# jank324/lynx

Hardware: AMD Instinct MI355X
Metric: particle-element-steps/sec (whole node) + achieved HBM GB/s, Segment.track ParticleBeam (higher is better)
Workload: dtype f32

## Files before the change

### lynx_amd/csrc/lynx_hip.hip

```cpp
#include <hip/hip_runtime.h>
#include <hip/hip_ext.h>
#include <rccl/rccl.h>

#include <algorithm>
#include <cstdio>
#include <cstdlib>
#include <cstring>
#include <map>
#include <mutex>
#include <string>
#include <type_traits>
#include <unordered_map>
#include <vector>

#include "lynx_device.hpp"
#include "lynx_grad.hpp"
#include "lynx_units.hpp"
#include "lynx_grad_units.hpp"
#include "lynx_trace.hpp"
#include "lynx_trace_grad.hpp"

using namespace lynx;

struct Knobs {
  int xpose = -1;
  int unroll = -1;
  int mom = -1;
  int min_tiles_per_wg = -1;
  int async_build = -1;
  int side_reduce = -1;
  int build_host_wait = -1;
  int gather_overlap = -1;
  int lanes_build_min_batch = 256;
  int piece = 8;
  int pair_levels_fused = 1;
  int merge_steps = 1;
  int reduce_ticket = 1;
  int one_round = -1;
  int track_units = 1;
  int unit_pairs = 1;
  int bwd_units = 1;
  int bwd_merge = 1;
  int bwd_pairs = 1;
  int build_in_tail = 1;
  int small_inline = -1;
  int bwd_reuse_table = 1;
  int host_visible_records = 1;
  int alternate_order = 1;
  int inline_pool = 1;
};

static void load_knobs(Knobs* k) {
  *k = Knobs();
  const struct { const char* name; int* value; } table[] = {
      {"LYNX_XPOSE", &k->xpose}, {"LYNX_UNROLL", &k->unroll}, {"LYNX_MOM", &k->mom},
      {"LYNX_MIN_TILES_PER_WG", &k->min_tiles_per_wg}, {"LYNX_ASYNC_BUILD", &k->async_build},
      {"LYNX_SIDE_REDUCE", &k->side_reduce}, {"LYNX_BUILD_HOST_WAIT", &k->build_host_wait},
      {"LYNX_GATHER_OVERLAP", &k->gather_overlap}, {"LYNX_LANES_BUILD_MIN_BATCH", &k->lanes_build_min_batch},
      {"LYNX_PIECE", &k->piece}, {"LYNX_PAIR_LEVELS_FUSED", &k->pair_levels_fused},
      {"LYNX_MERGE_STEPS", &k->merge_steps},
      {"LYNX_REDUCE_TICKET", &k->reduce_ticket}, {"LYNX_TRACK_UNITS", &k->track_units}, {"LYNX_ONE_ROUND", &k->one_round}, {"LYNX_UNIT_PAIRS", &k->unit_pairs}, {"LYNX_BWD_UNITS", &k->bwd_units},
      {"LYNX_BWD_MERGE", &k->bwd_merge}, {"LYNX_BWD_PAIRS", &k->bwd_pairs}, {"LYNX_BUILD_IN_TAIL", &k->build_in_tail},
      {"LYNX_SMALL_INLINE", &k->small_inline}, {"LYNX_INLINE_POOL", &k->inline_pool}, {"LYNX_ALTERNATE_ORDER", &k->alternate_order}, {"LYNX_HOST_VISIBLE_RECORDS", &k->host_visible_records}, {"LYNX_BWD_REUSE_TABLE", &k->bwd_reuse_table}};
  for (const auto& t : table) {
    const char* v = getenv(t.name);
    if (v && *v) *t.value = atoi(v);
  }
}
static inline int knob(int value, int dflt) { return value >= 0 ? value : dflt; }

struct lynx_ctx {
  Knobs knobs;
  int device = 0;
  hipStream_t stream = nullptr;
  hipStream_t s_build = nullptr;
  static constexpr int kTableSlots = 3;
  hipEvent_t ev_built[kTableSlots] = {}, ev_streamed_own[kTableSlots] = {}, ev_mark = nullptr;
  hipEvent_t ev_streamed[kTableSlots] = {};
  bool streamed_valid[kTableSlots] = {};
  unsigned seq = 0;
  bool main_dirty = false;
  bool main_idle = true;
  bool plain_events = false;
  unsigned long_calls = 0;
  struct FwdTable {
    const lynx_lattice* lat = nullptr;
    uint64_t version = 0;
    const void* energy = nullptr;
    int slot = -1;
    int merged = 0;
    bool units = false;
    size_t energy_bytes = 0;
    unsigned seq = 0;
    bool valid = false;
    void written(const void* dst, size_t bytes) {
      const char *a = (const char*)dst, *e = (const char*)energy;
      if (valid && a < e + energy_bytes && a + bytes > e) valid = false;
    }
  } fwd_table;
  const void* main_wrote = nullptr;
  std::mutex mu;
  void wrote(const void* dst, size_t bytes) {
    if (!dst || bytes == 0) return;
    std::lock_guard<std::mutex> lock(mu);
    fwd_table.written(dst, bytes);
  }
  hipEvent_t ev_start = nullptr, ev_stop = nullptr;
  int32_t* h_status = nullptr;
  int32_t* d_status = nullptr;
  unsigned int* d_tail_flag = nullptr;
  uint32_t tail_seq = 0;
  int can_wait_value = 0;
  std::string err;
  hipDeviceProp_t prop;
  std::multimap<size_t, void*> free_blocks;
  std::unordered_map<void*, size_t> live;
  std::vector<std::pair<const char*, size_t>> host_ranges;
  void* scratch_level = nullptr;
  size_t scratch_level_bytes = 0;
  unsigned int* scratch_tickets = nullptr;
  size_t scratch_tickets_count = 0;
  void* scratch_obs = nullptr;
  size_t scratch_obs_bytes = 0;
  void* scratch_erun = nullptr;
  size_t scratch_erun_bytes = 0;
  void* scratch_esteps = nullptr;
  size_t scratch_esteps_bytes = 0;
  int32_t* d_spec_valid = nullptr;
  void* scratch_products = nullptr;
  size_t scratch_products_bytes = 0;
  void* scratch_coefs = nullptr;
  size_t scratch_coefs_bytes = 0;
  static constexpr int kTableBwd = kTableSlots, kTablePb = kTableSlots + 1, kTableTrace = kTableSlots + 2;
  void* scratch_steps[kTableSlots + 3] = {};
  size_t scratch_steps_bytes[kTableSlots + 3] = {};
  void* scratch_trace[2] = {nullptr, nullptr};
  size_t scratch_trace_bytes[2] = {0, 0};
  void* scratch_trace_plan = nullptr;
  size_t scratch_trace_plan_bytes = 0;
  std::vector<int64_t> trace_plan;
  void* scratch_units_bwd[2] = {nullptr, nullptr};
  size_t scratch_units_bwd_bytes[2] = {0, 0};
  void* scratch_units[2 * kTableSlots] = {};
  size_t scratch_units_bytes[2 * kTableSlots] = {};
// ... 1014 lines not shown
      hipLaunchKernelGGL(k_pair_products, dim3((unsigned)groups, (unsigned)level.second), dim3(64), 0, stream,
                         lat->d_tasks + level.first, lat->batch, Bp, (double*)ctx->scratch_products);
      HIP_TRY(ctx, hipGetLastError());
    }
  }
  hipLaunchKernelGGL(k_emit_steps<T>, dim3((unsigned)groups, (unsigned)lat->n_steps), dim3(64), emit_steps_lds<T>(), stream, lv,
                     lat->d_step_slot, (const T*)d_energy_in, Bp, (const double*)ctx->scratch_products,
                     (const T*)ctx->scratch_coefs, merge_pairs, (T*)d_steps_out, (T*)d_energy_out,
                     d_units ? lat->d_step_unit[merge_pairs ? 1 : 0] : (const int32_t*)nullptr,
                     lat->units[merge_pairs ? 1 : 0].n_units, d_units, d_extras, se);
  HIP_TRY(ctx, hipGetLastError());
  return LYNX_OK;
}

template <typename T>
static int launch_build(lynx_ctx* ctx, lynx_lattice* lat, hipStream_t stream, const void* d_energy_in,
                        void* d_steps_out, void* d_energy_out, int merge_pairs = 0, bool underneath = false,
                        float* d_units = nullptr, float* d_extras = nullptr, bool force_lanes = false) {
  const bool lanes = lat->n_steps > 0 && (force_lanes || lat->batch >= ctx->knobs.lanes_build_min_batch);
  {
    const int rc = launch_cavity_flags<T>(ctx, lat, stream, d_energy_in, lanes);
    if (rc) return rc;
  }
  if (lanes) {
    const int rc = sync_pool(ctx, lat);
    return rc ? rc : launch_build_lanes<T>(ctx, lat, stream, d_energy_in, d_steps_out, d_energy_out, merge_pairs, d_units, d_extras);
  }
  int threads, chunk;
  build_shape<T>(ctx, lat, underneath, &threads, &chunk);
  const size_t lds = build_scratch_bytes(chunk, sizeof(T)) +
                     ((size_t)lat->n_steps * LYNX_STEP_STRIDE + lat->n_steps + 1) * sizeof(T);
  int rc;
  if (lat->prog_pool && ctx->knobs.inline_pool) {
    if ((size_t)lat->pool_count * sizeof(T) <= (size_t)kInlinePoolSmall) {
      if ((rc = allow_lds(ctx, k_build_inline<T, kInlinePoolSmall>, lds))) return rc;
      hipLaunchKernelGGL((k_build_inline<T, kInlinePoolSmall>), dim3((unsigned)lat->batch), dim3((unsigned)threads), lds, stream,
                         *reinterpret_cast<const InlinePool<kInlinePoolSmall>*>(&lat->h_pool), dev_view(lat),
                         (const T*)d_energy_in, (T*)d_steps_out, (T*)d_energy_out, chunk, merge_pairs);
    } else {
      if ((rc = allow_lds(ctx, k_build_inline<T, kInlinePoolLarge>, lds))) return rc;
      hipLaunchKernelGGL((k_build_inline<T, kInlinePoolLarge>), dim3((unsigned)lat->batch), dim3((unsigned)threads), lds, stream,
                         lat->h_pool, dev_view(lat), (const T*)d_energy_in, (T*)d_steps_out, (T*)d_energy_out, chunk, merge_pairs);
    }
  } else {
    if ((rc = sync_pool(ctx, lat)) || (rc = allow_lds(ctx, k_build<T>, lds))) return rc;
    hipLaunchKernelGGL(k_build<T>, dim3((unsigned)lat->batch), dim3((unsigned)threads), lds, stream, dev_view(lat),
                       (const T*)d_energy_in, (T*)d_steps_out, (T*)d_energy_out, chunk, merge_pairs);
  }
  HIP_TRY(ctx, hipGetLastError());
  if constexpr (sizeof(T) == 4) {
    if (d_units) {
      const UnitPlan& up = lat->units[merge_pairs ? 1 : 0];
      const int64_t n = lat->batch * up.n_units;
      hipLaunchKernelGGL(k_pack_units, dim3((unsigned)((n + 255) / 256)), dim3(256), 0, stream, up, lat->batch,
                         lat->n_steps, (const float*)d_steps_out, d_units, d_extras);
      HIP_TRY(ctx, hipGetLastError());
    }
  }
  return LYNX_OK;
}

int lynx_build_compose(lynx_ctx* ctx, lynx_lattice* lat, const void* d_energy_in, void* d_steps_out,
                       void* d_energy_out) {
  LYNX_NEED(ctx);
  ctx->main_idle = false;
  if (!ctx || !lat || !d_energy_in || !d_steps_out) return fail(ctx, LYNX_ERR_INVALID, "null argument");
  if (lat->batch > 0x7fffffffLL) return fail(ctx, LYNX_ERR_INVALID, "batch too large");
  HIP_TRY(ctx, use_device(ctx));
  ctx->main_dirty = true;
  const size_t es = dtype_size(lat->dtype);
  ctx->wrote(d_steps_out, (size_t)lat->batch * lat->n_steps * LYNX_STEP_STRIDE * es);
  ctx->wrote(d_energy_out, (size_t)lat->batch * es);
  return lat->dtype == LYNX_F64 ? launch_build<double>(ctx, lat, ctx->stream, d_energy_in, d_steps_out, d_energy_out)
                                : launch_build<float>(ctx, lat, ctx->stream, d_energy_in, d_steps_out, d_energy_out);
}


struct TrackPlan {
  hipEvent_t done = nullptr;
  bool full_cov;
  int unroll;
  int mom_mode;
  bool xpose;
  TrackArgs a;
  size_t lds;
  unsigned grid;
};

template <typename T>
static TrackPlan plan_track(lynx_ctx* ctx, const lynx_lattice* lat, int64_t B, int64_t N, int32_t S, bool moments,
                            bool full_cov) {
  TrackPlan p;
  p.full_cov = full_cov;
  constexpr int P = 16 / (int)sizeof(T);
  const int64_t cus = ctx->prop.multiProcessorCount > 0 ? ctx->prop.multiProcessorCount : 256;
  const Knobs& kn = ctx->knobs;
  const int64_t target = 512 * cus;
  p.mom_mode = knob(kn.mom, sizeof(T) == 4 ? 2 : 1);
  if (sizeof(T) == 8 || p.mom_mode < 2 || p.mom_mode > 3) p.mom_mode = sizeof(T) == 4 ? 2 : 1;
  p.a.n_particles = N;
  p.a.store = 0;
  p.a.tail_flag = nullptr;
  p.a.tail_seq = 0;
  p.a.tail_wg = 0;
  p.a.stash_offset = 0;
  p.a.reversed = 0;
  const bool single_map = S == 1 && lat && lat->h_steps[0].kind == LYNX_STEP_RUN &&
                          !(lat->h_steps[0].flags & LYNX_STEP_FLAG_OBSERVE);
  p.xpose = knob(kn.xpose, ((sizeof(T) == 8 || (single_map && !full_cov)) && N >= 8 * 64 * P) ? 1 : 0) != 0;
  int u = knob(kn.unroll, p.xpose ? P : (sizeof(T) == 4 ? (S > 1 ? 2 : 4) : 1));
  if (u != 1 && u != 2 && u != 4) u = 2;
  if (sizeof(T) == 8 && u > 2) u = 2;
  while (u > 1 && B * ((N + 256 * u - 1) / (256 * u)) < 4 * cus) u >>= 1;
  if (u != P) p.xpose = false;
  p.unroll = u;
  const int64_t tile = 256 * (int64_t)u;
  const int64_t ntiles = (N + tile - 1) / tile;
  int64_t min_tpw = std::max(1, knob(kn.min_tiles_per_wg, S > 1 ? 16 : 2));
  while (min_tpw > 1 && B * ((ntiles + min_tpw - 1) / min_tpw) < 4 * cus) --min_tpw;
  int64_t chunks = std::max<int64_t>(1, std::min<int64_t>((ntiles + min_tpw - 1) / min_tpw, (target + B - 1) / B));
  {
    const int64_t one_round = 3 * cus;
    const int cap = knob(kn.one_round, (S <= 1 && B * chunks > one_round && B * chunks <= 4 * one_round) ? 3 : 0);
    if (cap > 0) chunks = std::max<int64_t>(1, std::min<int64_t>(chunks, cap * cus / B));
  }
  int64_t tpw = (ntiles + chunks - 1) / chunks;
  chunks = (ntiles + tpw - 1) / tpw;
  p.a.chunks = (int32_t)chunks;
  p.a.tiles_per_wg = (int32_t)tpw;
  if (p.mom_mode == 2 && kn.mom < 0 && tpw * u <= 32) p.mom_mode = 3;
  if (p.mom_mode == 3 && tpw * u > 64) p.mom_mode = 2;
  size_t scratch = 4 * kPartialStride * sizeof(double);
  if (moments)
    scratch = std::max<size_t>(scratch, (size_t)(full_cov ? kMomSlabScalars : kMomSlabScalarsCompact) * (p.mom_mode >= 2 ? 4 : 8));
  if (p.xpose) scratch = std::max<size_t>(scratch, (size_t)(kTrackThreads / 64) * kWaveTileBytes);
  scratch = (scratch + 15) / 16 * 16;
  p.a.lds_scratch_bytes = (int32_t)scratch;
  p.a.n_observers = lat ? lat->n_observers : 0;
  p.lds = (scratch + ((size_t)S * LYNX_STEP_STRIDE + S + 1) * sizeof(T) + 7) / 8 * 8 + (size_t)2 * p.a.n_observers * 256 * sizeof(double);
  p.grid = (unsigned)(B * chunks);
  return p;
}

template <typename K, typename... Args>
static int launch_streaming(lynx_ctx* ctx, const TrackPlan& p, K kernel, size_t lds, const Args&... args) {
  int rc = allow_lds(ctx, kernel, lds);
  if (rc) return rc;
  hipEvent_t e0 = nullptr, e1 = p.done;
  if (ctx->profiling) {
    HIP_TRY(ctx, hipEventCreateWithFlags(&e0, timing_event_flags(ctx)));
    HIP_TRY(ctx, hipEventCreateWithFlags(&e1, timing_event_flags(ctx)));
  }
  hipExtLaunchKernelGGL(kernel, dim3(p.grid), dim3(kTrackThreads), (std::uint32_t)lds, ctx->stream, e0, e1, 0u, args...);
  HIP_TRY(ctx, hipGetLastError());
  if (ctx->profiling) ctx->prof_events.emplace_back(e0, e1);
  ctx->last_stream_stop = e1;
  return LYNX_OK;
}

template <typename T, int MOM, bool FULL, int UNROLL, bool XPOSE>
static int launch_direct_inst(lynx_ctx* ctx, const TrackPlan& p, const LatticeDev& lv, const void* d_energy_in,
                              const void* d_p_in, void* d_p_out, void* d_energy_out, const void* d_steps,
                              double* d_partials, double* d_obs) {
  return launch_streaming(ctx, p, k_track_direct<T, MOM, FULL, UNROLL, XPOSE>, p.lds, lv, p.a, (const T*)d_energy_in,
                          (const T*)d_p_in, (T*)d_p_out, (T*)d_energy_out, (const T*)d_steps, d_partials, d_obs);
}

#define LYNX_LAUNCH_ARGS ctx, p, lv, d_energy_in, d_p_in, d_p_out, d_energy_out, d_steps, d_partials, d_obs
#define LYNX_LAUNCH_PARAMS                                                                                     \
  lynx_ctx *ctx, const TrackPlan &p, const LatticeDev &lv, const void *d_energy_in, const void *d_p_in,        \
      void *d_p_out, void *d_energy_out, const void *d_steps, double *d_partials, double *d_obs

template <typename T, int MOM, bool FULL, int U>
static int launch_direct_mu(LYNX_LAUNCH_PARAMS) {
  if constexpr (U * 7 * sizeof(T) == 112) {
    if (p.xpose) return launch_direct_inst<T, MOM, FULL, U, true>(LYNX_LAUNCH_ARGS);
  }
  return launch_direct_inst<T, MOM, FULL, U, false>(LYNX_LAUNCH_ARGS);
}

template <typename T, int MOM, bool FULL>
static int launch_direct_m(LYNX_LAUNCH_PARAMS) {
  switch (p.unroll) {
    case 1: return launch_direct_mu<T, MOM, FULL, 1>(LYNX_LAUNCH_ARGS);
    case 2: return launch_direct_mu<T, MOM, FULL, 2>(LYNX_LAUNCH_ARGS);
    default:
      if constexpr (sizeof(T) == 4) return launch_direct_mu<T, MOM, FULL, 4>(LYNX_LAUNCH_ARGS);
      else return fail(ctx, LYNX_ERR_INVALID, "float64: at most 2 particles per lane");
  }
}

template <typename T>
static int launch_direct(LYNX_LAUNCH_PARAMS, bool moments) {
  const int mom = moments ? p.mom_mode : 0;
  if (mom == 0) return launch_direct_m<T, 0, false>(LYNX_LAUNCH_ARGS);
  if constexpr (sizeof(T) == 4) {
    if (mom == 3) return p.full_cov ? launch_direct_m<T, 3, true>(LYNX_LAUNCH_ARGS) : launch_direct_m<T, 3, false>(LYNX_LAUNCH_ARGS);
    return p.full_cov ? launch_direct_m<T, 2, true>(LYNX_LAUNCH_ARGS) : launch_direct_m<T, 2, false>(LYNX_LAUNCH_ARGS);
  } else {
    return p.full_cov ? launch_direct_m<T, 1, true>(LYNX_LAUNCH_ARGS) : launch_direct_m<T, 1, false>(LYNX_LAUNCH_ARGS);
  }
}
#undef LYNX_LAUNCH_ARGS
#undef LYNX_LAUNCH_PARAMS


static int proposed_class(const lynx_lattice* lat, int32_t first, int32_t last) {
  int rank = 1;
  for (int32_t e = first; e < last; ++e) {
    const lynx_elem& el = lat->h_elems[e];
    switch (el.kind) {
      case LYNX_KIND_IDENTITY:
      case LYNX_KIND_DRIFT:
      case LYNX_KIND_HCOR:
      case LYNX_KIND_VCOR:
      case LYNX_KIND_CAVITY:
      case LYNX_KIND_UNDULATOR: break;
      case LYNX_KIND_QUADRUPOLE: rank = std::max(rank, (el.flags & LYNX_FLAG_TILT) ? 3 : 1); break;
      case LYNX_KIND_DIPOLE: rank = std::max(rank, 2); break;
      default: rank = 3; break;
    }
  }
  return rank == 1 ? kClassU : rank == 2 ? kClassD : kClassDense;
}

static bool plan_units(const lynx_lattice* lat, bool merged, UnitPlan* plan) {
  const int32_t S = lat->n_steps;
  plan->n_units = 0;
  for (int32_t s = 0; s < S; ++s) {
    const lynx_step& st = lat->h_steps[s];
    if (st.flags & LYNX_STEP_FLAG_OBSERVE) return false;
    const bool pair = merged && s + 1 < S && st.kind == LYNX_STEP_RUN && lat->h_steps[s + 1].kind == LYNX_STEP_CAVITY;
    const int32_t last = pair ? lat->h_steps[s + 1].last : st.last;
    if (pair) ++s;
    if (plan->n_units >= kMaxUnits || s > 255) return false;
    const int u = plan->n_units++;
    plan->slot[u] = (unsigned char)s;
    plan->pair[u] = pair ? 1 : 0;
    plan->cls[u] = (unsigned char)proposed_class(lat, st.first, last);
  }
  for (int u = plan->n_units; u < kMaxUnits; ++u) plan->slot[u] = plan->cls[u] = plan->pair[u] = 0;
  return plan->n_units > 0;
}

static int ensure_units_plan(lynx_ctx* ctx, lynx_lattice* lat, bool merged) {
  const int m = merged ? 1 : 0;
  if (lat->units_made[m]) return LYNX_OK;
  UnitPlan& up = lat->units[m];
  lat->units_ok[m] = plan_units(lat, merged, &up) && lat->batch * up.n_units * kUnitStride < 0x7fffffffLL;
  lat->units_made[m] = true;
  if (!lat->units_ok[m]) return LYNX_OK;
  std::vector<int32_t> code((size_t)lat->n_steps, -1);
  for (int u = 0; u < up.n_units; ++u) code[up.slot[u]] = step_unit_code(u, up.cls[u], up.pair[u]);
  int rc;
  if (!lat->d_step_unit[m] && (rc = ctx_alloc(ctx, code.size() * sizeof(int32_t), (void**)&lat->d_step_unit[m]))) return rc;
  HIP_TRY(ctx, hipStreamSynchronize(ctx->s_build));
  HIP_TRY(ctx, sync_main(ctx));
  HIP_TRY(ctx, hipMemcpy(lat->d_step_unit[m], code.data(), code.size() * sizeof(int32_t), hipMemcpyHostToDevice));
  return LYNX_OK;
}

template <int MOM, bool FULL, int PAIRS, bool PAIR_FORM = false>
static int launch_units_inst(lynx_ctx* ctx, const TrackPlan& p, int32_t U, int32_t S, const void* d_p_in, void* d_p_out,
                             void* d_energy_out, const void* d_steps, const void* d_units, const void* d_extras,
                             double* d_partials) {
  const size_t lds = units_lds_bytes((size_t)p.a.lds_scratch_bytes, U);
  auto kernel = k_track_units<MOM, FULL, PAIRS>;
  if constexpr (PAIR_FORM) kernel = k_track_unit_pairs<MOM, FULL>;
  return launch_streaming(ctx, p, kernel, lds, p.a, U, S, (const float*)d_p_in, (float*)d_p_out, (float*)d_energy_out,
                          (const float*)d_steps, (const float*)d_units, (const float*)d_extras, d_partials);
}

static int launch_units(lynx_ctx* ctx, const TrackPlan& p, int32_t U, int32_t S, const void* d_p_in, void* d_p_out,
                        void* d_energy_out, const void* d_steps, const void* d_units, const void* d_extras,
                        double* d_partials, bool moments, bool pair_form) {
#define LYNX_UNITS_ARGS ctx, p, U, S, d_p_in, d_p_out, d_energy_out, d_steps, d_units, d_extras, d_partials
  if (pair_form)
    return moments ? launch_units_inst<3, false, 1, true>(LYNX_UNITS_ARGS) : launch_units_inst<0, false, 1, true>(LYNX_UNITS_ARGS);
  if (p.unroll == 4) {
    if (!moments) return launch_units_inst<0, false, 2>(LYNX_UNITS_ARGS);
    if (p.mom_mode == 3) return p.full_cov ? launch_units_inst<3, true, 2>(LYNX_UNITS_ARGS) : launch_units_inst<3, false, 2>(LYNX_UNITS_ARGS);
    return p.full_cov ? launch_units_inst<2, true, 2>(LYNX_UNITS_ARGS) : launch_units_inst<2, false, 2>(LYNX_UNITS_ARGS);
  }
  if (!moments) return launch_units_inst<0, false, 1>(LYNX_UNITS_ARGS);
  if (p.mom_mode == 3) return p.full_cov ? launch_units_inst<3, true, 1>(LYNX_UNITS_ARGS) : launch_units_inst<3, false, 1>(LYNX_UNITS_ARGS);
  return p.full_cov ? launch_units_inst<2, true, 1>(LYNX_UNITS_ARGS) : launch_units_inst<2, false, 1>(LYNX_UNITS_ARGS);
#undef LYNX_UNITS_ARGS
}

struct TrackTable {
  int slot = -1;
  bool async = false;
  bool tail = false;
  bool short_call = false;
  const void* d_steps = nullptr;
  const void* d_units = nullptr;
  const void* d_extras = nullptr;
  int n_units = 0;
  bool use_units = false;
};

template <typename T>
static int track_table(lynx_ctx* ctx, lynx_lattice* lat, int64_t B, int64_t N, int32_t S, const void* d_energy_in,
                       const void* d_energy_out, int flags, TrackPlan& p, TrackTable* t) {
  int rc;
  const int slot = t->slot = (int)(ctx->seq++ % (unsigned)lynx_ctx::kTableSlots);
  const size_t need = (size_t)B * S * LYNX_STEP_STRIDE * sizeof(T);
  if ((rc = ensure_scratch(ctx, &ctx->scratch_steps[slot], &ctx->scratch_steps_bytes[slot], need))) return rc;
  bool has_pair = false;
  for (int32_t s = 1; s < S; ++s)
    has_pair |= lat->h_steps[s].kind == LYNX_STEP_CAVITY && lat->h_steps[s - 1].kind == LYNX_STEP_RUN &&
                !(lat->h_steps[s - 1].flags & LYNX_STEP_FLAG_OBSERVE);
  p.a.merged_pairs = has_pair && sizeof(T) == 4 && p.unroll == 2 &&
                     !(flags & LYNX_TRACK_SEQUENTIAL_STEPS) && ctx->knobs.merge_steps;
  if (p.a.merged_pairs) {
    p.lds = (p.lds + 15) / 16 * 16;
    p.a.stash_offset = (int32_t)p.lds;
    p.lds += (size_t)kTrackThreads * 4 * sizeof(float);
  }
  const bool half_million = B * N >= (int64_t)512 << 10;
  t->short_call = half_million && (size_t)B * N * 7 * sizeof(T) < ((size_t)128 << 20) && !lat->has_cavity;
  bool inline_all = false;
  if (t->short_call && ctx->knobs.async_build < 0)
    inline_all = knob(ctx->knobs.small_inline, ctx->main_idle ? 1 : 0) != 0;
  const bool async = t->async = knob(ctx->knobs.async_build, half_million && !inline_all ? 1 : 0) != 0;
  hipStream_t bs = async ? ctx->s_build : ctx->stream;
  if (async) {
    if (ctx->streamed_valid[slot]) HIP_TRY(ctx, hipStreamWaitEvent(bs, ctx->ev_streamed[slot], 0));
    t->tail = ctx->can_wait_value && ctx->knobs.build_in_tail && !t->short_call;
    if (t->tail && ctx->tail_seq >= 2)
      HIP_TRY(ctx, hipStreamWaitValue32(bs, ctx->d_tail_flag, ctx->tail_seq - 1, hipStreamWaitValueGte, 0xffffffffu));
    if (ctx->main_dirty || (ctx->main_wrote && ctx->main_wrote == d_energy_in)) {
      HIP_TRY(ctx, hipEventRecord(ctx->ev_mark, ctx->stream));
      HIP_TRY(ctx, hipStreamWaitEvent(bs, ctx->ev_mark, 0));
      ctx->main_dirty = false;
      ctx->main_wrote = nullptr;
    }
  }
  float* d_units_w = nullptr;
  float* d_extras_w = nullptr;
  if constexpr (sizeof(T) == 4) {
    const int want_units = ctx->knobs.track_units;
    if (S > 1 && (p.unroll == 2 || p.unroll == 4) && !p.xpose && p.a.n_observers == 0 && want_units &&
        (uint64_t)N * 28u + ((uint64_t)1 << 20) < ((uint64_t)1 << 32)) {
      if ((rc = ensure_units_plan(ctx, lat, p.a.merged_pairs != 0))) return rc;
      t->use_units = lat->units_ok[p.a.merged_pairs ? 1 : 0];
    }
    if (want_units == 2 && !t->use_units)
      return fail(ctx, LYNX_ERR_INVALID, "LYNX_TRACK_UNITS=2: this call does not take the structured step loop");
    if (t->use_units) {
      const int64_t n = B * lat->units[p.a.merged_pairs ? 1 : 0].n_units;
      const int xs = lynx_ctx::kTableSlots + slot;
      if ((rc = ensure_scratch(ctx, &ctx->scratch_units[slot], &ctx->scratch_units_bytes[slot], (size_t)n * kUnitStride * sizeof(float))) ||
          (rc = ensure_scratch(ctx, &ctx->scratch_units[xs], &ctx->scratch_units_bytes[xs], (size_t)n * kUnitExtraStride * sizeof(float))))
        return rc;
      t->d_units = d_units_w = (float*)ctx->scratch_units[slot];
      t->d_extras = d_extras_w = (float*)ctx->scratch_units[xs];
      t->n_units = lat->units[p.a.merged_pairs ? 1 : 0].n_units;
    }
  }
  if ((rc = launch_build<T>(ctx, lat, bs, d_energy_in, ctx->scratch_steps[slot], nullptr, p.a.merged_pairs, async, d_units_w, d_extras_w)))
// ... 52 lines not shown
      rows = 0;
    } else {
      hipLaunchKernelGGL((k_reduce_moments<false, 256, kReduceStage>), dim3((unsigned)(B * groups)), dim3(256), lds, rs,
                         level_in, rows, rpg, groups, (double*)ctx->scratch_level);
      HIP_TRY(ctx, hipGetLastError());
      level_in = (const double*)ctx->scratch_level;
      rows = groups;
    }
  }
  if (rows > 0) {
    hipLaunchKernelGGL((k_reduce_moments<true, 256, kReduceStage>), dim3((unsigned)B), dim3(256), lds, rs, level_in,
                       rows, rows, 1, d_moments_out);
    HIP_TRY(ctx, hipGetLastError());
  }
  if (side) {
    {
      std::lock_guard<std::mutex> lock(ctx->mu);
      retire_side_ops(ctx, false);
    }
    HIP_TRY(ctx, hipEventRecord(ring->reduced, rs));
    ring->pending = true;
    side_op_issued(ctx, ring->reduced, d_moments_out, nullptr, false);
    ctx->side_wrote = d_moments_out;
  }
  return LYNX_OK;
}

template <typename T>
static int track_particles_t(lynx_ctx* ctx, lynx_lattice* lat, const LatticeDev& lv, int64_t B, int64_t N,
                             const void* d_energy_in, const void* d_p_in, void* d_p_out, void* d_energy_out,
                             double* d_moments_out, int flags, double* d_observations = nullptr) {
  const int32_t S = lv.n_steps;
  const bool moments = (flags & (LYNX_TRACK_MOMENTS | LYNX_TRACK_COVARIANCE)) != 0;
  const bool full_cov = (flags & LYNX_TRACK_COVARIANCE) != 0;
  TrackPlan p = plan_track<T>(ctx, lat, B, N, S, moments, full_cov);
  p.a.store = d_p_out ? 1 : 0;
  const bool shared_in = (flags & LYNX_TRACK_SHARED_INPUT) != 0;
  p.a.in_stride = shared_in ? 0 : N * 7;
  p.a.merged_pairs = 0;
  int rc;
  ctx->wrote(d_p_out, (size_t)B * N * 7 * sizeof(T));
  ctx->wrote(d_energy_out, (size_t)B * sizeof(T));
  ctx->wrote(d_moments_out, (size_t)B * LYNX_MOMENT_STRIDE * sizeof(double));
  ctx->wrote(d_observations, lat ? (size_t)B * lat->n_observers * 2 * sizeof(double) : 0);
  TrackTable t;
  if (S > 0 && (rc = track_table<T>(ctx, lat, B, N, S, d_energy_in, d_energy_out, flags, p, &t))) return rc;
  if ((int64_t)B * p.a.chunks > 0x7fffffffLL) return fail(ctx, LYNX_ERR_INVALID, "grid too large");
  double* d_partials = nullptr;
  lynx_ctx::PartialSlot* ring = nullptr;
  const bool side = moments && knob(ctx->knobs.side_reduce, (B * N >= (int64_t)512 << 10 && !t.short_call) ? 1 : 0) != 0;
  if (moments) {
    ring = &ctx->partial_ring[ctx->partial_seq++ % lynx_ctx::kPartialRing];
    if (ring->pending) {
      if (hipEventQuery(ring->reduced) != hipSuccess) HIP_TRY(ctx, hipEventSynchronize(ring->reduced));
      ring->pending = false;
    }
    const size_t need = (size_t)B * p.a.chunks * kPartialStride * sizeof(double);
    if ((rc = ensure_scratch(ctx, &ring->buf, &ring->bytes, need))) return rc;
    d_partials = (double*)ring->buf;
  }
  double* d_obs = nullptr;
  if (p.a.n_observers) {
    if (!d_observations) return fail(ctx, LYNX_ERR_INVALID, "the program has observer steps: d_observations required");
    const size_t need = (size_t)B * p.a.chunks * 2 * LYNX_MAX_OBSERVERS * sizeof(double);
    if ((rc = ensure_scratch(ctx, &ctx->scratch_obs, &ctx->scratch_obs_bytes, need))) return rc;
    d_obs = (double*)ctx->scratch_obs;
  }
  if (t.tail) {
    const int64_t cus = ctx->prop.multiProcessorCount > 0 ? ctx->prop.multiProcessorCount : 256;
    p.a.tail_flag = ctx->d_tail_flag;
    p.a.tail_seq = ++ctx->tail_seq;
    p.a.tail_wg = (int32_t)std::max<int64_t>(0, (int64_t)p.grid - 4 * cus);
  }
  if (!t.use_units && ctx->knobs.alternate_order &&
      (ctx->knobs.alternate_order == 2 || (size_t)B * N * 7 * sizeof(T) >= ((size_t)256 << 20)))
    p.a.reversed = ctx->knobs.alternate_order == 2 ? 1 : (int32_t)(ctx->long_calls++ & 1u);
  p.done = (t.slot >= 0 && t.async) ? ctx->ev_streamed_own[t.slot] : nullptr;
  if (side && !p.done) p.done = ring->track_done;
  if (t.use_units) {
    const UnitPlan& up = lat->units[p.a.merged_pairs ? 1 : 0];
    bool pair_form = ctx->knobs.unit_pairs != 0;
    for (int u = 0; u < up.n_units && pair_form; ++u) pair_form = up.cls[u] == kClassU && up.pair[u];
    pair_form = pair_form && p.unroll != 4 && (!moments || (p.mom_mode == 3 && !p.full_cov));
    if (ctx->knobs.unit_pairs == 2 && !pair_form)
      rc = fail(ctx, LYNX_ERR_INVALID, "LYNX_UNIT_PAIRS=2: this call does not take the kernel for lattices of [run, cavity] pairs");
    else
      rc = launch_units(ctx, p, t.n_units, S, d_p_in, d_p_out, d_energy_out, t.d_steps, t.d_units, t.d_extras, d_partials, moments, pair_form);
  } else {
    rc = launch_direct<T>(ctx, p, lv, d_energy_in, d_p_in, d_p_out, d_energy_out, t.d_steps, d_partials, d_obs, moments);
  }
  if (rc) {
    if (t.tail) --ctx->tail_seq;
    return rc;
  }
  if (p.a.n_observers) {
    hipLaunchKernelGGL(k_reduce_observers, dim3((unsigned)B), dim3(64), 0, ctx->stream, d_obs, p.a.chunks,
                       p.a.n_observers, (double)N, d_observations);
    HIP_TRY(ctx, hipGetLastError());
  }
  if (t.slot >= 0) {
    ctx->ev_streamed[t.slot] = ctx->last_stream_stop;
    ctx->streamed_valid[t.slot] = t.async && ctx->last_stream_stop != nullptr;
    if (!t.async) ctx->main_dirty = true;
  }
  if (d_energy_out) ctx->main_wrote = d_energy_out;
  if (moments) return reduce_moment_records(ctx, B, p.a.chunks, side, ring, d_partials, d_moments_out);
  return LYNX_OK;
}

int lynx_track_particles(lynx_ctx* ctx, lynx_lattice* lat, int64_t n_particles, const void* d_energy_in,
                         const void* d_p_in, void* d_p_out, void* d_energy_out, double* d_moments_out,
                         int flags, double* d_observations) {
  if (!ctx || !lat || !d_p_in) return fail(ctx, LYNX_ERR_INVALID, "null argument");
  if (n_particles <= 0) return fail(ctx, LYNX_ERR_INVALID, "n_particles must be > 0");
  if (lat->n_steps > 0 && !d_energy_in) return fail(ctx, LYNX_ERR_INVALID, "energy_in required");
  if ((flags & (LYNX_TRACK_MOMENTS | LYNX_TRACK_COVARIANCE)) && !d_moments_out)
    return fail(ctx, LYNX_ERR_INVALID, "LYNX_TRACK_MOMENTS / LYNX_TRACK_COVARIANCE need d_moments_out");
  if ((flags & LYNX_TRACK_SHARED_INPUT) && d_p_in == d_p_out)
    return fail(ctx, LYNX_ERR_INVALID, "a shared incoming beam cannot be tracked in place");
  HIP_TRY(ctx, use_device(ctx));
  LatticeDev lv = dev_view(lat);
  const int rc = lat->dtype == LYNX_F64
                     ? track_particles_t<double>(ctx, lat, lv, lat->batch, n_particles, d_energy_in, d_p_in, d_p_out,
                                                 d_energy_out, d_moments_out, flags, d_observations)
                     : track_particles_t<float>(ctx, lat, lv, lat->batch, n_particles, d_energy_in, d_p_in, d_p_out,
                                                d_energy_out, d_moments_out, flags, d_observations);
  ctx->main_idle = false;
  return rc;
}

int lynx_track_particles_new(lynx_ctx* ctx, lynx_lattice* lat, int64_t n_particles, const void* d_energy_in,
                             const void* d_p_in, int flags, int32_t want_energy_out, void** d_out ) {
  if (!ctx || !lat || !d_out) return fail(ctx, LYNX_ERR_INVALID, "null argument");
  for (int k = 0; k < 4; ++k) d_out[k] = nullptr;
  if (n_particles <= 0) return fail(ctx, LYNX_ERR_INVALID, "n_particles must be > 0");
  const size_t es = dtype_size(lat->dtype);
  const bool moments = (flags & (LYNX_TRACK_MOMENTS | LYNX_TRACK_COVARIANCE)) != 0;
  int rc = ctx_alloc(ctx, (size_t)lat->batch * (size_t)n_particles * 7 * es, &d_out[0]);
  if (!rc && want_energy_out) rc = ctx_alloc(ctx, (size_t)lat->batch * es, &d_out[1]);
  if (!rc && moments) {
    const size_t bytes = (size_t)lat->batch * LYNX_MOMENT_STRIDE * sizeof(double);
    if (bytes <= kHostVisibleMax && ctx->comm_ranks == 0 && ctx->knobs.host_visible_records) rc = ctx_alloc_host_visible(ctx, bytes, &d_out[2]);
    else rc = ctx_alloc(ctx, bytes, &d_out[2]);
  }
  if (!rc && lat->n_observers > 0) rc = ctx_alloc(ctx, (size_t)lat->batch * lat->n_observers * 2 * sizeof(double), &d_out[3]);
  if (!rc)
    rc = lynx_track_particles(ctx, lat, n_particles, d_energy_in, d_p_in, d_out[0], d_out[1], (double*)d_out[2], flags,
                              (double*)d_out[3]);
  if (rc) {
    const std::string why = ctx->err;
    (void)sync_main(ctx);
    for (int k = 0; k < 4; ++k) {
      if (d_out[k]) (void)ctx_free(ctx, d_out[k]);
      d_out[k] = nullptr;
    }
    ctx->err = why;
  }
  return rc;
}


static int ensure_bwd_tasks(lynx_ctx* ctx, lynx_lattice* lat) {
  if (lat->d_bwd_tasks) return LYNX_OK;
  std::vector<unsigned short> tasks;
  if (lat->n_elems >= 4096) return fail(ctx, LYNX_ERR_INVALID, "reverse pass: at most 4095 elements per program");
  for (int k = 1; k <= LYNX_KIND_UNDULATOR; ++k) {
    const int np = bwd_kind_params(k);
// ... 1342 lines not shown
```

### lynx_amd/csrc/lynx_units.hpp

```cpp
#pragma once

#include "lynx_device.hpp"
#include "lynx_unit_record.hpp"

namespace lynx {

__global__ __launch_bounds__(256) void k_pack_units(UnitPlan plan, int64_t B, int32_t S, const float* __restrict__ steps,
                                                    float* __restrict__ units, float* __restrict__ extras) {
  const int64_t i = (int64_t)blockIdx.x * blockDim.x + threadIdx.x;
  const int U = plan.n_units;
  if (i >= B * U) return;
  const int64_t b = i / U;
  const int u = (int)(i - b * U);
  const int slot = plan.slot[u];
  float pre[4] = {1.f, 0.f, 0.f, 1.f};
  if (plan.pair[u]) {
    const float* run = steps + (b * S + slot - 1) * LYNX_STEP_STRIDE;
    pre[0] = run[4]; pre[1] = run[5]; pre[2] = run[7 + 4]; pre[3] = run[7 + 5];
  }
  pack_unit_record<float>(steps + (b * S + slot) * LYNX_STEP_STRIDE, pre, slot, plan.cls[u], plan.pair[u],
                          units + i * kUnitStride, extras + i * kUnitExtraStride);
}


template <bool COMPLETE>
__device__ __forceinline__ void unit_kick(const float (&coef)[8], float sphi, lynx_f32x2 s_in, lynx_f32x2 d_in, lynx_f32x2& o4,
                                          lynx_f32x2& o5, float& widest) {
  const lynx_f32x2 d = -1.0f * s_in * coef[LYNX_C_BK];
  lynx_f32x2 dcos;
  if constexpr (COMPLETE) {
    dcos = cos_difference(d, coef[LYNX_C_PHI], sphi, coef[LYNX_C_COSPHI]);
  } else {
    dcos = cos_difference_small<lynx_f32x2>(d, sphi, coef[LYNX_C_COSPHI]);
    widest = __builtin_fmaxf(__builtin_fmaxf(__builtin_fabsf(d.x), __builtin_fabsf(d.y)), widest);
  }
  kick_outputs<lynx_f32x2>(coef, s_in, d_in, dcos, o4, o5);
}

template <int N>
__device__ __forceinline__ lynx_f32x2 row_dot(const float (&m)[N], const lynx_f32x2 (&v)[N]) {
  lynx_f32x2 acc = v[0] * m[0];
#pragma unroll
  for (int k = 1; k < N; ++k) acc = pk_fma(v[k], m[k], acc);
  return acc;
}

__device__ __forceinline__ bool pair_not_finite(const lynx_f32x2 (&z)[7]) {
  lynx_f32x2 acc = z[0] * 0.0f;
#pragma unroll
  for (int k = 1; k < 7; ++k) acc = pk_fma(z[k], 0.0f, acc);
  return (acc.x != acc.x) || (acc.y != acc.y);
}

__device__ __forceinline__ const float* particle_at(const float* base, uint32_t i) {
  return reinterpret_cast<const float*>(reinterpret_cast<const char*>(base) + i * 28u);
}
__device__ __forceinline__ float* particle_at(float* base, uint32_t i) {
  return reinterpret_cast<float*>(reinterpret_cast<char*>(base) + i * 28u);
}

__device__ __forceinline__ float in_vector_register(float uniform) {
  float v;
  asm volatile("v_mov_b32 %0, %1" : "=v"(v) : "s"(uniform));
  return v;
}

template <int MOM, bool FULL, int PAIRS> constexpr int units_waves_per_simd() {
  return PAIRS == 1 ? ((!FULL && (MOM == 0 || MOM == 3)) ? 5 : 1) : ((!FULL && (MOM == 0 || MOM == 3)) ? 4 : 1);
}

struct UnitHalf {
  float v[16];
};
__device__ __forceinline__ void unit_fetch(const float* __restrict__ half, UnitHalf& r) {
#pragma unroll
  for (int k = 0; k < 16; ++k) r.v[k] = uniform_value(half[k]);
}

template <int CLS>
__device__ __forceinline__ void unit_linear(const UnitHalf& map, const float* __restrict__ ex, lynx_f32x2 (&z)[7]) {
  const float* m = map.v;
  if constexpr (CLS == kClassU) {
    {
      const lynx_f32x2 v[3] = {z[0], z[1], z[6]};
      const float r0[3] = {m[0], m[1], m[2]}, r1[3] = {m[3], m[4], m[5]};
      const lynx_f32x2 o0 = row_dot<3>(r0, v), o1 = row_dot<3>(r1, v);
      z[0] = o0;
      z[1] = o1;
    }
    {
      const lynx_f32x2 v[3] = {z[2], z[3], z[6]};
      const float r2[3] = {m[6], m[7], m[8]}, r3[3] = {m[9], m[10], m[11]};
      const lynx_f32x2 o2 = row_dot<3>(r2, v), o3 = row_dot<3>(r3, v);
      z[2] = o2;
      z[3] = o3;
    }
    {
      const lynx_f32x2 v[2] = {z[4], z[5]};
      const float r4[2] = {m[12], m[13]}, r5[2] = {m[14], m[15]};
      const lynx_f32x2 o4 = row_dot<2>(r4, v), o5 = row_dot<2>(r5, v);
      z[4] = o4;
      z[5] = o5;
    }
  } else {
    static_assert(CLS == kClassD, "dense programs take units_dense_program");
    float md[8];
#pragma unroll
    for (int k = 0; k < 8; ++k) md[k] = uniform_value(ex[k]);
    const lynx_f32x2 vx[4] = {z[0], z[1], z[5], z[6]};
    const lynx_f32x2 vs[5] = {z[0], z[1], z[4], z[5], z[6]};
    const float r0[4] = {m[0], m[1], md[0], m[2]}, r1[4] = {m[3], m[4], md[1], m[5]};
    const float r4[5] = {md[2], md[3], m[12], m[13], md[4]}, r5[5] = {md[5], md[6], m[14], m[15], md[7]};
    const lynx_f32x2 o0 = row_dot<4>(r0, vx), o1 = row_dot<4>(r1, vx);
    const lynx_f32x2 o4 = row_dot<5>(r4, vs), o5 = row_dot<5>(r5, vs);
    {
      const lynx_f32x2 v[3] = {z[2], z[3], z[6]};
      const float r2[3] = {m[6], m[7], m[8]}, r3[3] = {m[9], m[10], m[11]};
      const lynx_f32x2 o2 = row_dot<3>(r2, v), o3 = row_dot<3>(r3, v);
      z[2] = o2;
      z[3] = o3;
    }
    z[0] = o0;
    z[1] = o1;
    z[4] = o4;
    z[5] = o5;
  }
}

template <bool COMPLETE>
__device__ __forceinline__ void unit_nonlinear(const UnitHalf& kick, int bits, lynx_f32x2 s_own, lynx_f32x2 d_own,
                                               lynx_f32x2 (&z)[7], float& widest) {
  if (bits & kUnitKick) {
    lynx_f32x2 s_in = s_own, d_in = d_own;
    if (bits & kUnitInverse) {
      const float* inv = kick.v + kUnitInv;
      s_in = pk_fma(z[5], inv[1], z[4] * inv[0]);
      d_in = pk_fma(z[5], inv[3], z[4] * inv[2]);
    }
    float coef[8];
#pragma unroll
    for (int k = 0; k < 8; ++k) coef[k] = kick.v[kUnitCoef + k];
    unit_kick<COMPLETE>(coef, kick.v[kUnitSinPhi], s_in, d_in, z[4], z[5], widest);
  }
}

__device__ __forceinline__ void unit_linear_dense(const float* __restrict__ tab, lynx_f32x2 (&z)[7]) {
  lynx_f32x2 o[7];
// ... 120 lines not shown
  const bool pairs_u = PAIR_FORM && units_all_pairs_u(U, g_units);
  LaneSums<T, MOM, FULL> sums;
  sums.init();
  T shift[6];
#pragma unroll
  for (int i = 0; i < 6; ++i) shift[i] = T(0);

  for (int it = 0; it < my_tiles; ++it) {
    const uint32_t tile = tile0 + (uint32_t)it;
    const uint32_t i0 = tile * kTile + tid;
    if (tile * kTile >= end) break;
    sums.begin_iteration();
    lynx_f32x2 z[PAIRS][7];
#pragma unroll
    for (int p = 0; p < PAIRS; ++p)
#pragma unroll
      for (int c = 0; c < 7; ++c) {
        z[p][c].x = zn[2 * p][c];
        z[p][c].y = zn[2 * p + 1][c];
      }
    if (it + 1 < my_tiles) {
      const uint32_t j0 = (tile + 1) * kTile + tid;
#pragma unroll
      for (int u = 0; u < UNROLL; ++u) {
        const uint32_t j = j0 + (uint32_t)u * kTrackThreads;
        load_particle(particle_at(src, j < end ? j : 0u), zn[u]);
      }
    }
    auto any_not_finite = [&]() {
      bool bad = false;
#pragma unroll
      for (int p = 0; p < PAIRS; ++p) bad = bad || pair_not_finite(z[p]);
      return __builtin_amdgcn_ballot_w64(bad) != 0;
    };
    bool all_dense = false;
    for (;;) {
      float widest = 0.f;
      if constexpr (PAIR_FORM) {
        if (__builtin_expect(pairs_u && !all_dense, 1)) units_program_pairs_u<PAIRS>(U, g_units, z, widest);
        else units_program<PAIRS, true>(U, g_units, g_extras, g_steps, all_dense, z, widest);
      } else {
        units_program<PAIRS, false>(U, g_units, g_extras, g_steps, all_dense, z, widest);
      }
      if (all_dense || !(any_not_finite() || __builtin_amdgcn_ballot_w64(widest > kCosDifferenceSmall) != 0)) break;
      all_dense = true;
#pragma unroll
      for (int u = 0; u < UNROLL; ++u) {
        const uint32_t i = i0 + (uint32_t)u * kTrackThreads;
        T t[7];
        load_particle(particle_at(src, i < end ? i : 0u), t);
#pragma unroll
        for (int c = 0; c < 7; ++c) {
          if (u % 2 == 0) z[u / 2][c].x = t[c];
          else z[u / 2][c].y = t[c];
        }
      }
    }

    T zo[UNROLL][7];
#pragma unroll
    for (int p = 0; p < PAIRS; ++p)
#pragma unroll
      for (int c = 0; c < 7; ++c) {
        zo[2 * p][c] = z[p][c].x;
        zo[2 * p + 1][c] = z[p][c].y;
      }
    if (MOM && it == 0) {
#pragma unroll
      for (int k = 0; k < 6; ++k) shift[k] = PAIR_FORM ? wave_first(zo[0][k]) : in_vector_register(wave_first(zo[0][k]));
    }
#pragma unroll
    for (int u = 0; u < UNROLL; ++u) {
      const uint32_t i = i0 + (uint32_t)u * kTrackThreads;
      if (i < end) {
        if (a.store) store_particle(particle_at(dst, i), zo[u]);
        if (MOM) sums.add(zo[u], shift);
      }
    }
    sums.end_iteration();
  }
  if (MOM) workgroup_moment_record<T, MOM, FULL>(sums, shift, smem_raw, partials + ((int64_t)b * a.chunks + chunk) * kPartialStride);
}

template <int MOM, bool FULL, int PAIRS>
__global__ __launch_bounds__(kTrackThreads, (units_waves_per_simd<MOM, FULL, PAIRS>())) void k_track_units(
    TrackArgs a, int32_t U, int32_t S, const float* p_in, float* p_out, float* __restrict__ energy_out,
    const float* __restrict__ steps_in, const float* __restrict__ units_in, const float* __restrict__ extras_in,
    double* __restrict__ partials) {
  track_units_body<MOM, FULL, PAIRS, false>(a, U, S, p_in, p_out, energy_out, steps_in, units_in, extras_in, partials);
}

template <int MOM, bool FULL>
__global__ __launch_bounds__(kTrackThreads) __attribute__((amdgpu_waves_per_eu(5, 5))) void k_track_unit_pairs(
    TrackArgs a, int32_t U, int32_t S, const float* p_in, float* p_out, float* __restrict__ energy_out,
    const float* __restrict__ steps_in, const float* __restrict__ units_in, const float* __restrict__ extras_in,
    double* __restrict__ partials) {
  track_units_body<MOM, FULL, 1, true>(a, U, S, p_in, p_out, energy_out, steps_in, units_in, extras_in, partials);
}

inline size_t units_lds_bytes(size_t slab_bytes, int ) { return slab_bytes; }

}
```

Baseline: 14070 billion.

## Stage unit-kernel particle I/O through per-wave LDS tiles with prefetch

Adds a tiled variant of the unit tracking kernels. Each wave loads its contiguous 64-particle spans with wide vector loads, transposes them through LDS into per-lane particles, prefetches the next tile, and writes results back through LDS using nontemporal vector stores. The aim is to replace strided 28-byte per-lane accesses with coalesced 16- and 12-byte accesses and to overlap loads with compute. It costs extra LDS per workgroup, which may lower occupancy. It also adds a knob that can disable the small-batch unroll and tile spreading.

Result: no change. 13950 billion (-0.8%).

```diff
diff --git a/lynx_amd/csrc/lynx_hip.hip b/lynx_amd/csrc/lynx_hip.hip
--- a/lynx_amd/csrc/lynx_hip.hip
+++ b/lynx_amd/csrc/lynx_hip.hip
@@ -39,6 +39,8 @@
   int one_round = -1;
   int track_units = 1;
   int unit_pairs = 1;
+  int unit_tiles = -1;
+  int spread_small = 1;
   int bwd_units = 1;
   int bwd_merge = 1;
   int bwd_pairs = 1;
@@ -59,7 +61,7 @@
       {"LYNX_GATHER_OVERLAP", &k->gather_overlap}, {"LYNX_LANES_BUILD_MIN_BATCH", &k->lanes_build_min_batch},
       {"LYNX_PIECE", &k->piece}, {"LYNX_PAIR_LEVELS_FUSED", &k->pair_levels_fused},
       {"LYNX_MERGE_STEPS", &k->merge_steps},
-      {"LYNX_REDUCE_TICKET", &k->reduce_ticket}, {"LYNX_TRACK_UNITS", &k->track_units}, {"LYNX_ONE_ROUND", &k->one_round}, {"LYNX_UNIT_PAIRS", &k->unit_pairs}, {"LYNX_BWD_UNITS", &k->bwd_units},
+      {"LYNX_REDUCE_TICKET", &k->reduce_ticket}, {"LYNX_TRACK_UNITS", &k->track_units}, {"LYNX_ONE_ROUND", &k->one_round}, {"LYNX_UNIT_PAIRS", &k->unit_pairs}, {"LYNX_UNIT_TILES", &k->unit_tiles}, {"LYNX_SPREAD_SMALL", &k->spread_small}, {"LYNX_BWD_UNITS", &k->bwd_units},
       {"LYNX_BWD_MERGE", &k->bwd_merge}, {"LYNX_BWD_PAIRS", &k->bwd_pairs}, {"LYNX_BUILD_IN_TAIL", &k->build_in_tail},
       {"LYNX_SMALL_INLINE", &k->small_inline}, {"LYNX_INLINE_POOL", &k->inline_pool}, {"LYNX_ALTERNATE_ORDER", &k->alternate_order}, {"LYNX_HOST_VISIBLE_RECORDS", &k->host_visible_records}, {"LYNX_BWD_REUSE_TABLE", &k->bwd_reuse_table}};
   for (const auto& t : table) {
@@ -1240,6 +1242,7 @@
   int unroll;
   int mom_mode;
   bool xpose;
+  bool unit_tiles = false;
   TrackArgs a;
   size_t lds;
   unsigned grid;
@@ -1269,13 +1272,13 @@
   int u = knob(kn.unroll, p.xpose ? P : (sizeof(T) == 4 ? (S > 1 ? 2 : 4) : 1));
   if (u != 1 && u != 2 && u != 4) u = 2;
   if (sizeof(T) == 8 && u > 2) u = 2;
-  while (u > 1 && B * ((N + 256 * u - 1) / (256 * u)) < 4 * cus) u >>= 1;
+  while (kn.spread_small && u > 1 && B * ((N + 256 * u - 1) / (256 * u)) < 4 * cus) u >>= 1;
   if (u != P) p.xpose = false;
   p.unroll = u;
   const int64_t tile = 256 * (int64_t)u;
   const int64_t ntiles = (N + tile - 1) / tile;
   int64_t min_tpw = std::max(1, knob(kn.min_tiles_per_wg, S > 1 ? 16 : 2));
-  while (min_tpw > 1 && B * ((ntiles + min_tpw - 1) / min_tpw) < 4 * cus) --min_tpw;
+  while (kn.spread_small && min_tpw > 1 && B * ((ntiles + min_tpw - 1) / min_tpw) < 4 * cus) --min_tpw;
   int64_t chunks = std::max<int64_t>(1, std::min<int64_t>((ntiles + min_tpw - 1) / min_tpw, (target + B - 1) / B));
   {
     const int64_t one_round = 3 * cus;
@@ -1418,13 +1421,13 @@
   return LYNX_OK;
 }
 
-template <int MOM, bool FULL, int PAIRS, bool PAIR_FORM = false>
+template <int MOM, bool FULL, int PAIRS, bool PAIR_FORM = false, bool TILES = false>
 static int launch_units_inst(lynx_ctx* ctx, const TrackPlan& p, int32_t U, int32_t S, const void* d_p_in, void* d_p_out,
                              void* d_energy_out, const void* d_steps, const void* d_units, const void* d_extras,
                              double* d_partials) {
-  const size_t lds = units_lds_bytes((size_t)p.a.lds_scratch_bytes, U);
-  auto kernel = k_track_units<MOM, FULL, PAIRS>;
-  if constexpr (PAIR_FORM) kernel = k_track_unit_pairs<MOM, FULL>;
+  const size_t lds = units_lds_bytes((size_t)p.a.lds_scratch_bytes, TILES);
+  auto kernel = k_track_units<MOM, FULL, PAIRS, TILES>;
+  if constexpr (PAIR_FORM) kernel = k_track_unit_pairs<MOM, FULL, TILES>;
   return launch_streaming(ctx, p, kernel, lds, p.a, U, S, (const float*)d_p_in, (float*)d_p_out, (float*)d_energy_out,
                           (const float*)d_steps, (const float*)d_units, (const float*)d_extras, d_partials);
 }
@@ -1433,8 +1436,15 @@
                         void* d_energy_out, const void* d_steps, const void* d_units, const void* d_extras,
                         double* d_partials, bool moments, bool pair_form) {
 #define LYNX_UNITS_ARGS ctx, p, U, S, d_p_in, d_p_out, d_energy_out, d_steps, d_units, d_extras, d_partials
+  if (pair_form && p.unit_tiles)
+    return moments ? launch_units_inst<3, false, 1, true, true>(LYNX_UNITS_ARGS) : launch_units_inst<0, false, 1, true, true>(LYNX_UNITS_ARGS);
   if (pair_form)
     return moments ? launch_units_inst<3, false, 1, true>(LYNX_UNITS_ARGS) : launch_units_inst<0, false, 1, true>(LYNX_UNITS_ARGS);
+  if (p.unit_tiles) {
+    if (!moments) return launch_units_inst<0, false, 1, false, true>(LYNX_UNITS_ARGS);
+    if (p.mom_mode == 3) return p.full_cov ? launch_units_inst<3, true, 1, false, true>(LYNX_UNITS_ARGS) : launch_units_inst<3, false, 1, false, true>(LYNX_UNITS_ARGS);
+    return p.full_cov ? launch_units_inst<2, true, 1, false, true>(LYNX_UNITS_ARGS) : launch_units_inst<2, false, 1, false, true>(LYNX_UNITS_ARGS);
+  }
   if (p.unroll == 4) {
     if (!moments) return launch_units_inst<0, false, 2>(LYNX_UNITS_ARGS);
     if (p.mom_mode == 3) return p.full_cov ? launch_units_inst<3, true, 2>(LYNX_UNITS_ARGS) : launch_units_inst<3, false, 2>(LYNX_UNITS_ARGS);
@@ -1653,7 +1663,15 @@
     bool pair_form = ctx->knobs.unit_pairs != 0;
     for (int u = 0; u < up.n_units && pair_form; ++u) pair_form = up.cls[u] == kClassU && up.pair[u];
     pair_form = pair_form && p.unroll != 4 && (!moments || (p.mom_mode == 3 && !p.full_cov));
-    if (ctx->knobs.unit_pairs == 2 && !pair_form)
+    constexpr int64_t kUnitTilesMinWhole = 8;
+    const int want_tiles = ctx->knobs.unit_tiles;
+    const bool planner_tiles = N >= kUnitTilesMinWhole * 512;
+    p.unit_tiles = p.unroll == 2 && ((want_tiles < 0 || want_tiles == 3) ? planner_tiles : want_tiles != 0);
+    if (want_tiles == 2 && !p.unit_tiles)
+      rc = fail(ctx, LYNX_ERR_INVALID, "LYNX_UNIT_TILES=2: this call does not hold two particles per lane, which the wave tiles of the unit kernels need");
+    else if (want_tiles == 3 && !p.unit_tiles)
+      rc = fail(ctx, LYNX_ERR_INVALID, "LYNX_UNIT_TILES=3: the planner does not pick the wave tiles of the unit kernels for this call");
+    else if (ctx->knobs.unit_pairs == 2 && !pair_form)
       rc = fail(ctx, LYNX_ERR_INVALID, "LYNX_UNIT_PAIRS=2: this call does not take the kernel for lattices of [run, cavity] pairs");
     else
       rc = launch_units(ctx, p, t.n_units, S, d_p_in, d_p_out, d_energy_out, t.d_steps, t.d_units, t.d_extras, d_partials, moments, pair_form);
diff --git a/lynx_amd/csrc/lynx_units.hpp b/lynx_amd/csrc/lynx_units.hpp
--- a/lynx_amd/csrc/lynx_units.hpp
+++ b/lynx_amd/csrc/lynx_units.hpp
@@ -63,6 +63,33 @@
   float v;
   asm volatile("v_mov_b32 %0, %1" : "=v"(v) : "s"(uniform));
   return v;
+}
+
+constexpr int kSpanDwords = 64 * 7;
+constexpr int kUnitTileLdsBytes = (kTrackThreads / 64) * 2 * kSpanDwords * 4;
+typedef unsigned int lynx_u32x3 __attribute__((ext_vector_type(3)));
+typedef unsigned int lynx_u32x3u __attribute__((ext_vector_type(3), aligned(4)));
+struct SpanRegs {
+  lynx_u32x4 a;
+  lynx_u32x3 b;
+};
+__device__ __forceinline__ void span_fetch(const float* span, uint32_t lane, SpanRegs& r) {
+  const char* g = reinterpret_cast<const char*>(span);
+  r.a = *reinterpret_cast<const lynx_u32x4u*>(g + lane * 16u);
+  r.b = *reinterpret_cast<const lynx_u32x3u*>(g + 1024 + lane * 12u);
+}
+__device__ __forceinline__ void span_store(float* span, uint32_t lane, const SpanRegs& r) {
+  char* g = reinterpret_cast<char*>(span);
+  __builtin_nontemporal_store(r.a, reinterpret_cast<lynx_u32x4u*>(g + lane * 16u));
+  __builtin_nontemporal_store(r.b, reinterpret_cast<lynx_u32x3u*>(g + 1024 + lane * 12u));
+}
+__device__ __forceinline__ void span_to_lds(unsigned int* s_span, int lane, const SpanRegs& r) {
+  *reinterpret_cast<lynx_u32x4*>(s_span + 4 * lane) = r.a;
+  *reinterpret_cast<lynx_u32x3u*>(s_span + 256 + 3 * lane) = r.b;
+}
+__device__ __forceinline__ void span_from_lds(const unsigned int* s_span, int lane, SpanRegs& r) {
+  r.a = *reinterpret_cast<const lynx_u32x4*>(s_span + 4 * lane);
+  r.b = *reinterpret_cast<const lynx_u32x3u*>(s_span + 256 + 3 * lane);
 }
 
 template <int MOM, bool FULL, int PAIRS> constexpr int units_waves_per_simd() {
@@ -349,22 +376,196 @@
   if (MOM) workgroup_moment_record<T, MOM, FULL>(sums, shift, smem_raw, partials + ((int64_t)b * a.chunks + chunk) * kPartialStride);
 }
 
-template <int MOM, bool FULL, int PAIRS>
+template <int MOM, bool FULL, bool PAIR_FORM>
+__device__ __forceinline__ void track_units_body_tiles(
+    const TrackArgs& a, int32_t U, int32_t S, const float* p_in, float* p_out, float* __restrict__ energy_out,
+    const float* __restrict__ steps_in, const float* __restrict__ units_in, const float* __restrict__ extras_in,
+    double* __restrict__ partials) {
+  using T = float;
+  constexpr int UNROLL = 2;
+  extern __shared__ __attribute__((aligned(16))) unsigned char smem_raw[];
+  announce_tail(a);
+  const int tid = threadIdx.x;
+  const int64_t b = __builtin_amdgcn_readfirstlane((int)(blockIdx.x / a.chunks));
+  const int chunk = __builtin_amdgcn_readfirstlane((int)(blockIdx.x % a.chunks));
+  const uint32_t end = (uint32_t)a.n_particles;
+  constexpr uint32_t kTile = (uint32_t)kTrackThreads * UNROLL;
+  const T* src = p_in + b * a.in_stride;
+  T* dst = p_out + b * (int64_t)a.n_particles * 7;
+  const float* g_steps = steps_in + b * (int64_t)S * LYNX_STEP_STRIDE;
+  const float* g_units = units_in + b * (int64_t)U * kUnitStride;
+  const float* g_extras = extras_in + b * (int64_t)U * kUnitExtraStride;
+
+  const uint32_t tile0 = (uint32_t)chunk * (uint32_t)a.tiles_per_wg;
+  const int my_tiles = a.tiles_per_wg;
+  if (energy_out && chunk == 0 && tid == 0 && S > 0) energy_out[b] = g_steps[(S - 1) * LYNX_STEP_STRIDE + LYNX_ENERGY_OFFSET];
+
+  const bool pairs_u = PAIR_FORM && units_all_pairs_u(U, g_units);
+  LaneSums<T, MOM, FULL> sums;
+  sums.init();
+  T shift[6];
+#pragma unroll
+  for (int i = 0; i < 6; ++i) shift[i] = T(0);
+
+  auto lane_afresh = [&]() {
+    int t = tid;
+    asm volatile("" : "+v"(t));
+    return t & 63;
+  };
+  const int wave = __builtin_amdgcn_readfirstlane(tid >> 6);
+  unsigned int* s_wave = reinterpret_cast<unsigned int*>(smem_raw) + wave * (2 * kSpanDwords);
+  auto whole_tile = [&](uint32_t tile) { return (tile + 1) * kTile <= end; };
+  SpanRegs sn[2];
+  auto fetch_spans = [&](uint32_t tile, int lane) {
+    const uint32_t first = tile * kTile + (uint32_t)wave * 64u;
+    span_fetch(particle_at(src, first), (uint32_t)lane, sn[0]);
+    span_fetch(particle_at(src, first + kTrackThreads), (uint32_t)lane, sn[1]);
+  };
+  auto run_units = [&](uint32_t i0, lynx_f32x2 (&z)[1][7]) {
+    bool all_dense = false;
+    for (;;) {
+      float widest = 0.f;
+      if constexpr (PAIR_FORM) {
+        if (__builtin_expect(pairs_u && !all_dense, 1)) units_program_pairs_u<1>(U, g_units, z, widest);
+        else units_program<1, true>(U, g_units, g_extras, g_steps, all_dense, z, widest);
+      } else {
+        units_program<1, false>(U, g_units, g_extras, g_steps, all_dense, z, widest);
+      }
+      const bool bad = pair_not_finite(z[0]) || widest > kCosDifferenceSmall;
+      if (all_dense || __builtin_amdgcn_ballot_w64(bad) == 0) break;
+      all_dense = true;
+#pragma unroll
+      for (int u = 0; u < 2; ++u) {
+        uint32_t i = i0 + (uint32_t)u * kTrackThreads;
+        asm volatile("" : "+v"(i));
+        T t[7];
+        load_particle(particle_at(src, i < end ? i : 0u), t);
+#pragma unroll
+        for (int c = 0; c < 7; ++c) {
+          if (u == 0) z[0][c].x = t[c];
+          else z[0][c].y = t[c];
+        }
+      }
+    }
+  };
+  int it = 0;
+  if (my_tiles > 0 && whole_tile(tile0)) {
+    fetch_spans(tile0, lane_afresh());
+    for (; it < my_tiles && whole_tile(tile0 + (uint32_t)it); ++it) {
+      const uint32_t tile = tile0 + (uint32_t)it;
+      sums.begin_iteration();
+      lynx_f32x2 z[1][7];
+      {
+        const int lane = lane_afresh();
+        wave_fence();
+        span_to_lds(s_wave, lane, sn[0]);
+        span_to_lds(s_wave + kSpanDwords, lane, sn[1]);
+        wave_fence();
+        const unsigned int* s_mine = s_wave + 7 * lane;
+#pragma unroll
+        for (int c = 0; c < 7; ++c) {
+          z[0][c].x = __uint_as_float(s_mine[c]);
+          z[0][c].y = __uint_as_float(s_mine[kSpanDwords + c]);
+          asm volatile("");
+        }
+        const bool more = it + 1 < my_tiles && whole_tile(tile + 1);
+        fetch_spans(more ? tile + 1 : tile, lane);
+      }
+      run_units(tile * kTile + tid, z);
+      if (MOM && it == 0) {
+#pragma unroll
+        for (int k = 0; k < 6; ++k) shift[k] = PAIR_FORM ? wave_first(z[0][k].x) : in_vector_register(wave_first(z[0][k].x));
+      }
+      if (a.store) {
+        const int lane = lane_afresh();
+        unsigned int* s_mine = s_wave + 7 * lane;
+#pragma unroll
+        for (int c = 0; c < 7; ++c) {
+          s_mine[c] = __float_as_uint(z[0][c].x);
+          s_mine[kSpanDwords + c] = __float_as_uint(z[0][c].y);
+        }
+        wave_fence();
+        const uint32_t first = tile * kTile + (uint32_t)wave * 64u;
+#pragma unroll
+        for (int h = 0; h < 2; ++h) {
+          SpanRegs r;
+          span_from_lds(s_wave + h * kSpanDwords, lane, r);
+          span_store(particle_at(dst, first + (uint32_t)h * kTrackThreads), (uint32_t)lane, r);
+        }
+      }
+      if (MOM) {
+        T zo[2][7];
+#pragma unroll
+        for (int c = 0; c < 7; ++c) {
+          zo[0][c] = z[0][c].x;
+          zo[1][c] = z[0][c].y;
+        }
+        sums.add(zo[0], shift);
+        sums.add(zo[1], shift);
+      }
+      sums.end_iteration();
+    }
+  }
+  if (it < my_tiles && (tile0 + (uint32_t)it) * kTile < end) {
+    const uint32_t i0 = (tile0 + (uint32_t)it) * kTile + tid;
+    sums.begin_iteration();
+    lynx_f32x2 z[1][7];
+#pragma unroll
+    for (int u = 0; u < 2; ++u) {
+      const uint32_t i = i0 + (uint32_t)u * kTrackThreads;
+      T t[7];
+      load_particle(particle_at(src, i < end ? i : 0u), t);
+#pragma unroll
+      for (int c = 0; c < 7; ++c) {
+        if (u == 0) z[0][c].x = t[c];
+        else z[0][c].y = t[c];
+      }
+    }
+    run_units(i0, z);
+    T zo[2][7];
+#pragma unroll
+    for (int c = 0; c < 7; ++c) {
+      zo[0][c] = z[0][c].x;
+      zo[1][c] = z[0][c].y;
+    }
+    if (MOM && it == 0) {
+#pragma unroll
+      for (int k = 0; k < 6; ++k) shift[k] = PAIR_FORM ? wave_first(zo[0][k]) : in_vector_register(wave_first(zo[0][k]));
+    }
+#pragma unroll
+    for (int u = 0; u < 2; ++u) {
+      const uint32_t i = i0 + (uint32_t)u * kTrackThreads;
+      if (i < end) {
+        if (a.store) store_particle(particle_at(dst, i), zo[u]);
+        if (MOM) sums.add(zo[u], shift);
+      }
+    }
+    sums.end_iteration();
+  }
+  if (MOM) workgroup_moment_record<T, MOM, FULL>(sums, shift, smem_raw, partials + ((int64_t)b * a.chunks + chunk) * kPartialStride);
+}
+
+template <int MOM, bool FULL, int PAIRS, bool TILES = false>
 __global__ __launch_bounds__(kTrackThreads, (units_waves_per_simd<MOM, FULL, PAIRS>())) void k_track_units(
     TrackArgs a, int32_t U, int32_t S, const float* p_in, float* p_out, float* __restrict__ energy_out,
     const float* __restrict__ steps_in, const float* __restrict__ units_in, const float* __restrict__ extras_in,
     double* __restrict__ partials) {
-  track_units_body<MOM, FULL, PAIRS, false>(a, U, S, p_in, p_out, energy_out, steps_in, units_in, extras_in, partials);
-}
-
-template <int MOM, bool FULL>
+  static_assert(!TILES || PAIRS == 1, "wave tiles: two particles per lane");
+  if constexpr (TILES) track_units_body_tiles<MOM, FULL, false>(a, U, S, p_in, p_out, energy_out, steps_in, units_in, extras_in, partials);
+  else track_units_body<MOM, FULL, PAIRS, false>(a, U, S, p_in, p_out, energy_out, steps_in, units_in, extras_in, partials);
+}
+
+template <int MOM, bool FULL, bool TILES = false>
 __global__ __launch_bounds__(kTrackThreads) __attribute__((amdgpu_waves_per_eu(5, 5))) void k_track_unit_pairs(
     TrackArgs a, int32_t U, int32_t S, const float* p_in, float* p_out, float* __restrict__ energy_out,
     const float* __restrict__ steps_in, const float* __restrict__ units_in, const float* __restrict__ extras_in,
     double* __restrict__ partials) {
-  track_units_body<MOM, FULL, 1, true>(a, U, S, p_in, p_out, energy_out, steps_in, units_in, extras_in, partials);
-}
-
-inline size_t units_lds_bytes(size_t slab_bytes, int ) { return slab_bytes; }
-
-}
+  if constexpr (TILES) track_units_body_tiles<MOM, FULL, true>(a, U, S, p_in, p_out, energy_out, steps_in, units_in, extras_in, partials);
+  else track_units_body<MOM, FULL, 1, true>(a, U, S, p_in, p_out, energy_out, steps_in, units_in, extras_in, partials);
+}
+
+inline size_t units_lds_bytes(size_t slab_bytes, bool tiles) {
+  return tiles ? (slab_bytes > (size_t)kUnitTileLdsBytes ? slab_bytes : (size_t)kUnitTileLdsBytes) : slab_bytes;
+}
+
+}
```
